# willSapgreen/stereo-vision

Measured on AMD Instinct MI355X. Metric: stereo pairs/sec (ELAS 1242x375, ROBOTICS, D1+D2+LR), higher is better.
Workload: dtype u8

## Files before the change

### include/svh.h

```cpp
#ifndef SVH_H
#define SVH_H

#include <stddef.h>
#include <stdint.h>

#ifdef __cplusplus
extern "C" {
#endif

#define SVH_OK                 0
#define SVH_ERR_FEW_SUPPORT    1
#define SVH_ERR_BAD_ARG       -1
#define SVH_ERR_HIP           -2
#define SVH_ERR_UNSUPPORTED   -3
#define SVH_ERR_NO_DEVICE     -4
#define SVH_ERR_BAD_DIMS      -7

typedef struct svh_elas_params {
    int32_t disp_min;
    int32_t disp_max;
    float   support_threshold;
    int32_t support_texture;
    int32_t candidate_stepsize;
    int32_t incon_window_size;
// ... 103 lines not shown
                                      uint64_t* first_ticket);
int32_t svh_elas_stream_pop_n(svh_elas_stream* s, int32_t n, int32_t* status, int32_t* popped);
int32_t svh_elas_stream_push_n(svh_elas_stream* s, int32_t n, const uint8_t* const* I1, const uint8_t* const* I2,
                               float* const* D1, float* const* D2, uint64_t* first_ticket);

#define SVH_DISP_F32 0
#define SVH_DISP_U16 1
#define SVH_MAPS_BOTH 0
#define SVH_MAPS_LEFT 1
typedef struct { int32_t format; int32_t maps; } svh_elas_output;
int32_t svh_elas_process_out(svh_elas* e, const uint8_t* I1, const uint8_t* I2, void* D1, void* D2,
                             const int32_t* dims, const svh_elas_output* out);
int32_t svh_elas_process_batch_out(svh_elas* e, int32_t n, const uint8_t* const* I1, const uint8_t* const* I2,
                                   void* const* D1, void* const* D2, const int32_t* dims, int32_t* status,
                                   const svh_elas_output* out);
svh_elas_stream* svh_elas_stream_open_out(svh_elas* e, const int32_t* dims, int32_t depth, const svh_elas_output* out);
int32_t svh_elas_stream_push_out(svh_elas_stream* s, const uint8_t* I1, const uint8_t* I2, void* D1, void* D2,
                                 uint64_t* ticket);
int32_t svh_elas_stream_push_out_n(svh_elas_stream* s, int32_t n, const uint8_t* const* I1, const uint8_t* const* I2,
                                   void* const* D1, void* const* D2, uint64_t* first_ticket);
int32_t svh_disparity_pack_u16(const float* D, int32_t d_on_device, int64_t n, uint16_t* out, int32_t out_on_device);
int32_t svh_disparity_unpack_u16(const uint16_t* v, int64_t n, float* out);

int64_t svh_elas_trim(void);

int32_t svh_elas_set_lanes(int32_t lanes);
int32_t svh_elas_set_queue_plan(int32_t plan);
int32_t svh_elas_get_queue_plan(int32_t* plan, int32_t* streams_per_lane, int32_t* classes);
int32_t svh_elas_set_group(int32_t pairs);

int32_t svh_elas_set_stage(int32_t where);
void svh_elas_stage_stats(int64_t* device_groups, int64_t* handed_back);
void svh_elas_sizing_stats(int64_t* out4);
void svh_elas_get_settings(int32_t out[4]);

enum svh_elas_stage {
    SVH_ELAS_DESC1 = 0,
    SVH_ELAS_DESC2,
    SVH_ELAS_DCAN_RAW,
    SVH_ELAS_SUPPORT,
    SVH_ELAS_TRI1,
    SVH_ELAS_TRI2,
    SVH_ELAS_PLANES1,
    SVH_ELAS_PLANES2,
    SVH_ELAS_GRID1,
    SVH_ELAS_GRID2,
    SVH_ELAS_D1_RAW,
    SVH_ELAS_D2_RAW,
    SVH_ELAS_D1_LR,
    SVH_ELAS_D2_LR,
    SVH_ELAS_D1_SEG,
    SVH_ELAS_D2_SEG,
    SVH_ELAS_D1_GAP,
    SVH_ELAS_D2_GAP,
    SVH_ELAS_STAGE_COUNT
};
int32_t svh_elas_set_taps(svh_elas* e, int32_t enable);
int32_t svh_elas_get_stage(svh_elas* e, int32_t stage, void* buf, size_t cap, size_t* size);

int32_t svh_elas_last_timing(svh_elas* e, const char** names, float* ms, int32_t cap);

int32_t svh_profile_enable(int32_t on);
void    svh_profile_only(const char* kernel);
void    svh_profile_reset(void);
int32_t svh_profile_get(int32_t index, const char** name, double* total_ms, int64_t* launches);

// ... 178 lines not shown
```

### stereo-vision_amd/csrc/elas_engine.cpp

```cpp
#include <hip/hip_runtime.h>
#include <stdio.h>
#include <string.h>

#include <atomic>
#include <chrono>
#include <condition_variable>
#include <deque>
#include <functional>
#include <algorithm>
#include <map>
#include <memory>
#include <mutex>
#include <string>
#include <thread>
#include <vector>

#include "hip_guard.h"
#include "queue_plan.h"
#include "svh_internal.h"

namespace svh {

static thread_local int t_device = 0;

#define HIP_TRY(kind, expr) SVH_HIP_TRY(nullptr, kind, expr)
#define LANE_GROW(buf, bytes) SVH_HIP_GROW(nullptr, buf, bytes)

struct KernelStat {
    double total_ms = 0;
    int64_t launches = 0;
};
static std::mutex g_prof_mu;
static std::map<std::string, KernelStat> g_prof;
static std::atomic<int> g_prof_on{0};
static char g_prof_only[64] = "";

struct EventProfiler : Profiler {
    hipStream_t stream = nullptr;
    std::vector<hipEvent_t> ev;
    std::vector<const char*> names;
    size_t used = 0;
    bool skipping = false;
    void begin(const char* kernel) override {
        skipping = g_prof_only[0] && strcmp(kernel, g_prof_only) != 0;
        if (skipping) return;
        if (ev.size() < 2 * (used + 1)) {
            hipEvent_t a, b;
            if (hipEventCreate(&a) != hipSuccess || hipEventCreate(&b) != hipSuccess) return;
            ev.push_back(a);
// ... 36 lines not shown

static int queue_cap();
static int worker_count();

struct LaneBufs {
    HipBuf<uint8_t> img;
    HipBuf<uint8_t> desc;
    HipBuf<int16_t> dcan;
    HipBuf<int32_t> owner;
    HipBuf<uint8_t> prior_dev;
    HipBuf<TriRaster> raster;
    HipBuf<float> planes;
    HipBuf<uint32_t> seed, mask;
    HipBuf<uint16_t> lists;
    HipBuf<float> Draw;
    HipBuf<float> D;
    HipBuf<float> tmp;
    HipBuf<uint16_t> U;
    HipBuf<int32_t> labels, counts;
    HipBuf<int32_t> seg_nroots;
    HipBuf<uint8_t> stage_blob;
    PinnedBuf<int16_t> h_dcan;
    PinnedBuf<uint8_t> h_img, h_prior;
    PinnedBuf<StageCounts> h_counts;
};

struct Lane : LaneBufs {
    EventProfiler prof;
    int device = 0;
    hipStream_t stream = nullptr, stage_stream = nullptr, post_stream = nullptr;
    hipStream_t cls_stream[QC_COUNT] = {nullptr, nullptr, nullptr};
    int plan_req = QP_AUTO;
    int parity = 0;
    bool qp_known = false;
    QueuePlan qp{};
    int prio_least = 0, prio_greatest = 0;
    bool split = false;
    hipEvent_t a_ev = nullptr, b_ev = nullptr;
    hipEvent_t wait_ev = nullptr;
    hipStream_t copy_stream = nullptr;
    hipEvent_t match_ev = nullptr, copy_ev = nullptr;
    bool poll_wait = false;
    bool parallel_host = true;
    bool lone_group = true;
    int32_t W = 0, H = 0, disp_max = -1, step = 0, grid_size = 0, sub = -1, gcap = 0;
    Dims d{};
    bool desc_fly = false;
    int64_t owner_hi = 0;
    size_t prior_cap = 0;
    size_t ntri_max = 0;
    std::vector<HostPrior> hp;
    std::vector<int32_t> P;
    StageDev stg{};
    bool stage_ok = false;
    hipEvent_t stage_ev = nullptr;
    bool resident = false;
    bool force_host = false;
    float P_key[5] = {-1, -1, -1, -1, -1};
    static constexpr int kHist = 4;
    int32_t hist_sup[kHist] = {}, hist_tri[kHist] = {};
    int hist_n = 0, hist_at = 0;
    int32_t hist_g = 0;
    svh_elas_params hist_p{};
    PhaseBSize sized{};
    size_t o_P = 0, o_sup = 0, o_tri = 0;

    void release() {
        if (!stream) return;
        (void)hipSetDevice(device);
        static_cast<LaneBufs&>(*this) = LaneBufs();
        stage_ok = false; stg = StageDev{};
        P_key[0] = -1;
        hist_n = 0;
        W = H = 0;
    }

    void destroy() {
        if (!cls_stream[QC_NORMAL] && !cls_stream[QC_HIGH] && !cls_stream[QC_LOW]) return;
        (void)hipSetDevice(device);
        release();
        for (hipEvent_t* e : {&wait_ev, &match_ev, &copy_ev, &stage_ev, &a_ev, &b_ev})
            if (*e) {
                (void)hipEventDestroy(*e);
                *e = nullptr;
            }
        for (hipEvent_t e : prof.ev) (void)hipEventDestroy(e);
        prof.ev.clear();
        prof.names.clear();
        if (copy_stream) (void)hipStreamDestroy(copy_stream);
        for (hipStream_t& cs : cls_stream)
            if (cs) {
                (void)hipStreamDestroy(cs);
                cs = nullptr;
            }
        copy_stream = stream = stage_stream = post_stream = nullptr;
    }

    int bind_streams() {
        if (!qp_known) {
            HIP_TRY(none, hipSetDevice(device));
            if (hipDeviceGetStreamPriorityRange(&prio_least, &prio_greatest) != hipSuccess) {
                (void)hipGetLastError();
                prio_least = prio_greatest = 0;
            }
            qp = make_queue_plan(prio_least, prio_greatest, queue_cap(), worker_count(), plan_req);
            qp_known = true;
        }
        const QueueLane& ql = qp.lane[parity & 1];
        for (int k = 0; k < ql.nstreams; k++) {
            hipStream_t& cs = cls_stream[ql.cls[k]];
            if (cs) continue;
            HIP_TRY(none, hipSetDevice(device));
            if (qp.plan == QP_ONE)
                HIP_TRY(none, hipStreamCreateWithFlags(&cs, hipStreamNonBlocking));
            else
                HIP_TRY(none, hipStreamCreateWithPriority(&cs, hipStreamNonBlocking,
                                                          queue_priority_of(ql.cls[k], prio_least, prio_greatest)));
        }
        stream = cls_stream[ql.cls[ql.phase_stream[QPH_A]]];
        stage_stream = cls_stream[ql.cls[ql.phase_stream[QPH_S]]];
        post_stream = cls_stream[ql.cls[ql.phase_stream[QPH_B]]];
        return SVH_OK;
    }

    int ensure(const svh_elas_params& p, int32_t w, int32_t h, int32_t g) {
        if (int rc = bind_streams()) return rc;
        const int32_t st = p.candidate_stepsize + (p.subsampling ? p.candidate_stepsize % 2 : 0);
        if (w == W && h == H && p.disp_max == disp_max && st == step && p.grid_size == grid_size &&
            p.subsampling == sub && g <= gcap)
            return SVH_OK;
        release();
        d = make_dims(p, w, h);
        const size_t N = (size_t)w * h, DN = (size_t)d.DW * d.DH, G2 = (size_t)2 * g;
        LANE_GROW(img, G2 * N);
        LANE_GROW(desc, G2 * N * 16);
        LANE_GROW(owner, G2 * N * sizeof(int32_t));
        HIP_TRY(copy, hipMemset(owner, 0, G2 * N * sizeof(int32_t)));
        owner_hi = svh::env("SVH_TEST_OWNER_HI") ? atoll(svh::env("SVH_TEST_OWNER_HI")) : 0;
        LANE_GROW(Draw, G2 * DN * sizeof(float));
        LANE_GROW(D, G2 * DN * sizeof(float));
        LANE_GROW(tmp, G2 * DN * sizeof(float));
        LANE_GROW(labels, G2 * DN * sizeof(int32_t));
        LANE_GROW(counts, G2 * DN * sizeof(int32_t));
        LANE_GROW(seg_nroots, G2 * (size_t)((d.DW + 63) / 64) * ((d.DH + 15) / 16) * sizeof(int32_t));
        const size_t nc = (size_t)d.Wc * d.Hc;
        LANE_GROW(dcan, g * nc * sizeof(int16_t));
        LANE_GROW(h_dcan, g * nc * sizeof(int16_t));
        LANE_GROW(h_img, G2 * N);
        const size_t nsup = nc + 6;
        ntri_max = 2 * nsup + 8;
// ... 24 lines not shown
            LANE_GROW(stage_blob, off);
            HIP_TRY(copy, hipMemset(stage_blob, 0, off));
            LANE_GROW(h_counts, sizeof(StageCounts));
            uint8_t* b = stage_blob;
            stg.dcan = dcan;
            stg.sup_raw = reinterpret_cast<int32_t*>(b + a_sup);
            stg.counts = reinterpret_cast<StageCounts*>(b + a_cnt);
            stg.ids = reinterpret_cast<int32_t*>(b + a_ids);
            stg.xys = reinterpret_cast<int32_t*>(b + a_xys);
            stg.nbr = reinterpret_cast<uint32_t*>(b + a_nbr);
            int32_t** ia[6] = {&stg.pxy, &stg.buck, &stg.buck2, &stg.byx, &stg.order, &stg.oxy};
            uint32_t** ua[4] = {&stg.lx, &stg.ly, &stg.tmp, &stg.P};
            for (int k = 0; k < 6; k++) *ia[k] = reinterpret_cast<int32_t*>(b + a_arr[k]);
            for (int k = 0; k < 4; k++) *ua[k] = reinterpret_cast<uint32_t*>(b + a_arr[6 + k]);
            stg.dmap = reinterpret_cast<int32_t*>(b + a_arr[10]);
            stg.fl = reinterpret_cast<uint32_t*>(b + a_fl);
            stg.fr = reinterpret_cast<uint32_t*>(b + a_fr);
            stg.wl = reinterpret_cast<int32_t*>(b + a_wl);
            stg.cntw = reinterpret_cast<uint32_t*>(b + a_cw);
            stg.sup_cap = (int32_t)cap;
            stg.rec_cap = (int32_t)rec;
            stage_ok = true;
        }
        HIP_TRY(wait, hipDeviceSynchronize());
        W = w; H = h; disp_max = p.disp_max; step = st; grid_size = p.grid_size; sub = p.subsampling;
        gcap = g;
        return SVH_OK;
    }
};

static std::atomic<int> g_wait_us{40};
static std::atomic<bool> g_hostprof{false};
static hipError_t lane_wait(Lane& L) {
    if (!L.poll_wait || g_wait_us <= 0) return hipStreamSynchronize(L.stream);
    if (!L.wait_ev) {
        hipError_t e = hipEventCreateWithFlags(&L.wait_ev, hipEventDisableTiming);
        if (e != hipSuccess) return e;
    }
    hipError_t e = hipEventRecord(L.wait_ev, L.stream);
    if (e != hipSuccess) return e;
    for (;;) {
        e = hipEventQuery(L.wait_ev);
        if (e != hipErrorNotReady) return e;
        std::this_thread::sleep_for(std::chrono::microseconds(g_wait_us.load(std::memory_order_relaxed)));
    }
}

struct Pool {
    std::mutex mu;
    std::condition_variable cv;
    std::vector<Lane*> lanes;
    std::vector<Lane*> free_list;
    int max_lanes = 4;
    int queue_plan = -2;
};

static std::mutex g_mu;

static std::map<int, Pool*>& g_pools = *new std::map<int, Pool*>();
static std::atomic<int> g_lanes{6};
static std::atomic<int> g_group{32};
static std::atomic<bool> g_group_set{false};
static std::atomic<int> g_stage_mode{-1};
static int stage_mode_from_env();
static std::atomic<int> g_queue_plan{QP_AUTO};
static std::atomic<int> g_queue_cap{kQueueCapDefault};
static int queue_cap() { return g_queue_cap.load(); }
static int worker_count() { return g_lanes.load(); }
static void apply_config(const svh_config& c, int explicit_call) {
    if (explicit_call) {
        if (c.elas_workers > 0) svh_elas_set_lanes(c.elas_workers);
        if (c.elas_pairs_per_launch > 0) svh_elas_set_group(c.elas_pairs_per_launch);
        svh_elas_set_stage(c.elas_stage);
        if (c.wait_us >= 0) g_wait_us = c.wait_us;
    }
    if (const char* e = svh::env("SVH_WAIT_US")) g_wait_us = atoi(e);
    if (svh::env("SVH_STAGE")) g_stage_mode.store(stage_mode_from_env());
    g_hostprof = svh::env("SVH_HOST_PROF") != nullptr;
    g_queue_cap = queue_cap_from_text(getenv("GPU_MAX_HW_QUEUES"));
    if (const char* e = svh::env("SVH_QUEUE_PLAN")) {
        const int v = atoi(e);
        g_queue_plan = v >= 0 && v <= QP_LAST ? v : QP_AUTO;
    }
}
namespace { struct ConfigHook { ConfigHook() { svh::on_config(apply_config); } } g_config_hook; }
static int group_for(size_t N) {
    const int g = std::max(1, std::min(g_group.load(), kMaxGroup));
    if (g_group_set.load()) return g;
    size_t a = std::max<size_t>(1, std::min<size_t>(g, (size_t)32 * 1024 * 1024 / std::max<size_t>(N, 1)));
    size_t free_b = 0, total_b = 0;
    if (a > 1 && hipMemGetInfo(&free_b, &total_b) == hipSuccess && free_b > 0) {
        const size_t per_pair = 120 * std::max<size_t>(N, 1), sets = (size_t)2 * std::max(1, g_lanes.load());
        a = std::max<size_t>(1, std::min<size_t>(a, free_b / 2 / (per_pair * sets)));
    } else {
        (void)hipGetLastError();
    }
    return (int)a;
}

static Pool* pool_for(int device) {
    std::lock_guard<std::mutex> lk(g_mu);
    auto it = g_pools.find(device);
    if (it != g_pools.end()) return it->second;
    Pool* p = new Pool();
    g_pools[device] = p;
    return p;
}

static void acquire_lanes(int device, int count, Lane** out) {
    Pool* p = pool_for(device);
    std::unique_lock<std::mutex> lk(p->mu);
    p->max_lanes = 2 * g_lanes.load() + 2;
    for (;;) {
        const int can_make = p->max_lanes - (int)p->lanes.size();
        if ((int)p->free_list.size() + std::max(can_make, 0) >= count) {
            for (int i = 0; i < count; i++) {
                if (!p->free_list.empty()) {
                    out[i] = p->free_list.back();
                    p->free_list.pop_back();
                } else {
                    Lane* l = new Lane();
                    l->device = device;
                    l->plan_req = p->queue_plan != -2 ? p->queue_plan : g_queue_plan.load();
                    p->lanes.push_back(l);
                    out[i] = l;
                }
                out[i]->parity = i;
            }
            return;
        }
        p->cv.wait(lk);
    }
}

static Lane* acquire_lane(int device) {
    Lane* l = nullptr;
    acquire_lanes(device, 1, &l);
    return l;
}

static void release_lane(Lane* l) {
    Pool* p = pool_for(l->device);
    {
        std::lock_guard<std::mutex> lk(p->mu);
        p->free_list.push_back(l);
    }
    p->cv.notify_all();
}

struct Taps {
    bool enabled = false;
    std::vector<uint8_t> data[SVH_ELAS_STAGE_COUNT];
};

}

struct svh_elas {
    svh_elas_params p;
    int device;
    svh::Taps taps;
    std::vector<std::string> tnames;
    std::vector<float> tms;
};

namespace svh {

struct GroupIO {
    int32_t g;
    bool in_device;
    const uint8_t* dI[2];
    size_t in_stride;
    const uint8_t* const* hI[2];
    int32_t pitch;
    bool out_device;
    float* dD[2];
    size_t out_stride;
    float* const* hD[2];
    int32_t format = SVH_DISP_F32;
// ... 39 lines not shown
static std::atomic<uint64_t> g_hp_ns[HP_N];
static std::atomic<uint64_t> g_hp_pairs{0};
static uint64_t cpu_ns() {
    timespec ts;
    clock_gettime(CLOCK_THREAD_CPUTIME_ID, &ts);
    return (uint64_t)ts.tv_sec * 1000000000ull + ts.tv_nsec;
}
struct HostProfDump {
    ~HostProfDump() {
        if (!g_hostprof || !g_hp_pairs) return;
        static const char* nm[HP_N] = {"enqueue A", "waits", "filters", "delaunay", "pack", "enqueue B"};
        double tot = 0;
        for (int i = 0; i < HP_N; i++) tot += g_hp_ns[i];
        fprintf(stderr, "[svh host prof] %llu pairs, %.1f us cpu/pair:", (unsigned long long)g_hp_pairs.load(),
                tot / 1e3 / g_hp_pairs);
        for (int i = 0; i < HP_N; i++) fprintf(stderr, "  %s %.1f", nm[i], g_hp_ns[i] / 1e3 / g_hp_pairs);
        fprintf(stderr, "\n");
    }
};
static HostProfDump g_hp_dump;
#define HP_MARK(slot) do { if (g_hostprof) { uint64_t n_ = cpu_ns(); g_hp_ns[slot] += n_ - hp_t; hp_t = n_; } } while (0)

static int stage_mode_from_env() {
    const char* e = svh::env("SVH_STAGE");
    if (!e || !*e || !strcmp(e, "auto") || !strcmp(e, "-1")) return -1;
    if (!strcmp(e, "host") || !strcmp(e, "0")) return 0;
    if (!strcmp(e, "device") || !strcmp(e, "1")) return 1;
    fprintf(stderr, "svhip: SVH_STAGE=%s is not one of auto|-1, host|0, device|1: using auto\n", e);
    return -1;
}

static std::atomic<int64_t> g_stage_dev_groups{0}, g_stage_redo_groups{0};
static std::atomic<int64_t> g_sized_bound{0}, g_sized_hist{0}, g_short_tri{0}, g_short_sup{0};

static hipError_t event_wait(Lane& L, hipEvent_t ev) {
    if (!L.poll_wait || g_wait_us <= 0) return hipEventSynchronize(ev);
    for (;;) {
        hipError_t e = hipEventQuery(ev);
        if (e != hipErrorNotReady) return e;
        std::this_thread::sleep_for(std::chrono::microseconds(g_wait_us.load(std::memory_order_relaxed)));
    }
}

static int run_group_body(Lane& L, const svh_elas_params& p, const int32_t* dims, const GroupIO& io,
                          int32_t* status, Taps* taps, svh_elas* timing, int mode, int prefer_device);

static int run_group(Lane& L, const svh_elas_params& p, const int32_t* dims, const GroupIO& io,
                     int32_t* status, Taps* taps, svh_elas* timing, int mode = RG_ALL, int prefer_device = 0) {
    const int rc = run_group_body(L, p, dims, io, status, taps, timing, mode, prefer_device);
    if (rc == SVH_ERR_HIP) {
        const std::string keep = svh_last_error();
        for (hipStream_t cs : L.cls_stream)
            if (cs) (void)hipStreamSynchronize(cs);
        L.split = false;
        if (L.copy_stream) (void)hipStreamSynchronize(L.copy_stream);
        (void)hipGetLastError();
        L.prof.used = 0;
        L.resident = false;
        L.force_host = false;
        L.P_key[0] = -1;
        fail(rc, keep);
    }
    return rc;
}

static int run_group_body(Lane& L, const svh_elas_params& p, const int32_t* dims, const GroupIO& io,
                          int32_t* status, Taps* taps, svh_elas* timing, int mode, int prefer_device) {
    const int32_t W = dims[0], H = dims[1], g = io.g;
    int rc = check_params(p, W, H);
    if (rc) return rc;
    if (g < 1 || g > kMaxGroup) return fail(SVH_ERR_BAD_ARG, "bad group size");
    HIP_TRY(none, hipSetDevice(L.device));
    rc = L.ensure(p, W, H, g);
    if (rc) return rc;
    if (g > 1) taps = nullptr;
    const Dims& d = L.d;
    const bool u16 = !io.out_device && io.format == SVH_DISP_U16;
    const int nmaps = !io.out_device && io.maps == SVH_MAPS_LEFT ? 1 : 2;
    const size_t DNu = ((size_t)d.DW * d.DH + 7) & ~(size_t)7;
    if (u16) LANE_GROW(L.U, (size_t)L.gcap * 2 * DNu * sizeof(uint16_t));
    hipStream_t s = L.stream, ss = s, sb = L.split ? L.post_stream : s;
    const bool prof_on = g_prof_on.load() != 0;
    PhaseProfiler prof_a(&L.prof, s), prof_s(&L.prof, s), prof_b(&L.prof, sb);
    const LaunchCtx cx = {s, prof_on ? &prof_a : nullptr, L.lone_group};
    LaunchCtx cx_s = cx, cx_b = {sb, prof_on ? &prof_b : nullptr, L.lone_group};
    const size_t N = (size_t)W * H, DN = (size_t)d.DW * d.DH;
    const size_t nc = (size_t)d.Wc * d.Hc;
// ... 582 lines not shown
}

void svh_profile_reset(void) {
    std::lock_guard<std::mutex> lk(g_prof_mu);
    g_prof.clear();
}

int32_t svh_profile_get(int32_t index, const char** name, double* total_ms, int64_t* launches) {
    std::lock_guard<std::mutex> lk(g_prof_mu);
    if (index < 0) return (int32_t)g_prof.size();
    int32_t i = 0;
    for (auto& kv : g_prof) {
        if (i++ == index) {
            if (name) *name = kv.first.c_str();
            if (total_ms) *total_ms = kv.second.total_ms;
            if (launches) *launches = kv.second.launches;
            return SVH_OK;
        }
    }
    return SVH_ERR_BAD_ARG;
}

int64_t svh_elas_trim(void) {
    int64_t freed = 0;
    std::vector<Pool*> pools;
    {
        std::lock_guard<std::mutex> lk(g_mu);
        for (auto& kv : g_pools) pools.push_back(kv.second);
    }
    for (Pool* p : pools) {
        std::vector<Lane*> idle;
        {
            std::lock_guard<std::mutex> lk(p->mu);
            idle.swap(p->free_list);
            for (Lane* l : idle) p->lanes.erase(std::find(p->lanes.begin(), p->lanes.end(), l));
        }
        for (Lane* l : idle) {
            l->destroy();
            delete l;
            freed++;
        }
        p->cv.notify_all();
    }
    return freed;
}

int32_t svh_elas_set_lanes(int32_t lanes) {
    if (lanes < 1) lanes = 1;
    if (lanes > 64) lanes = 64;
    g_lanes.store(lanes);
    return lanes;
}

void svh_elas_params_default(svh_elas_params* p, int32_t setting) {
    const bool rob = setting == SVH_ELAS_ROBOTICS;
    p->disp_min = 0;
    p->disp_max = 255;
    p->support_threshold = rob ? 0.85f : 0.95f;
    p->support_texture = 10;
    p->candidate_stepsize = 5;
    p->incon_window_size = 5;
    p->incon_threshold = 5;
    p->incon_min_support = 5;
    p->add_corners = rob ? 0 : 1;
    p->grid_size = 20;
    p->beta = 0.02f;
    p->gamma = rob ? 3.f : 5.f;
// ... 72 lines not shown
    rc = run_group(*L, e->p, dims, io, &st, &e->taps, e);
    release_lane(L);
    if (rc == SVH_ERR_HIP) report_hip_failure("svh_elas_process");
    return rc ? rc : st;
}

int32_t svh_elas_process(svh_elas* e, const uint8_t* I1, const uint8_t* I2, float* D1, float* D2,
                         const int32_t* dims) {
    if (!e || !I1 || !I2 || !D1 || !D2 || !dims) return fail(SVH_ERR_BAD_ARG, "null argument");
    return process_impl(e, I1, I2, D1, D2, dims, SVH_DISP_F32, SVH_MAPS_BOTH);
}

int32_t svh_elas_process_out(svh_elas* e, const uint8_t* I1, const uint8_t* I2, void* D1, void* D2,
                             const int32_t* dims, const svh_elas_output* out) {
    int32_t format, maps;
    if (!output_form(out, &format, &maps)) return fail(SVH_ERR_BAD_ARG, "bad output format / map selection");
    if (!e || !I1 || !I2 || !D1 || (!D2 && maps == SVH_MAPS_BOTH) || !dims) return fail(SVH_ERR_BAD_ARG, "null argument");
    return process_impl(e, I1, I2, static_cast<float*>(D1), static_cast<float*>(D2), dims, format, maps);
}

static int32_t batch_impl(svh_elas* e, int32_t n, const int32_t* dims, int32_t* status,
                          const std::function<GroupIO(int32_t, int32_t)>& io_of) {
    int32_t rc = require_device(e->device);
    if (rc) return rc;
    rc = check_params(e->p, dims[0], dims[1]);
    if (rc) return rc;
    const int32_t G = group_for((size_t)dims[0] * dims[1]);
    const int32_t ngroups = (n + G - 1) / G;
    const int lanes = std::min<int>(g_lanes.load(), ngroups);
    const int deep = n >= 32 ? 2 : 1;
    std::vector<int32_t> st(n, SVH_OK);
    std::vector<int32_t> grc(ngroups, SVH_OK);
    std::vector<std::string> errs(std::max(lanes, 1));
    auto worker = [&](int w) {
        Lane* slot[2] = {nullptr, nullptr};
        acquire_lanes(e->device, ngroups > 1 ? 2 : 1, slot);
        for (Lane* L : slot)
            if (L) {
                L->parallel_host = ngroups <= lanes;
                L->lone_group = ngroups == 1;
                L->poll_wait = !L->parallel_host;
                if (hipSetDevice(L->device) == hipSuccess) (void)L->ensure(e->p, dims[0], dims[1], G);
            }
        struct Job { int32_t gi = -1; GroupIO io{}; int32_t first = 0; };
        int32_t my_next = w;
        auto take = [&]() {
            Job j;
            const int32_t gi = my_next;
            my_next += lanes;
            if (gi < ngroups) {
                j.gi = gi;
                j.first = gi * G;
                j.io = io_of(j.first, std::min(G, n - j.first));
            }
            return j;
        };
        auto note = [&](const Job& j, int rcj) {
            if (rcj != SVH_OK && grc[j.gi] == SVH_OK) {
                grc[j.gi] = rcj;
                if (rcj < 0) errs[w] = svh_last_error();
            }
        };
        Job pending[2];
        Job cur = take();
        int k = 0;
        if (cur.gi >= 0) note(cur, run_group(*slot[0], e->p, dims, cur.io, &st[cur.first], nullptr, nullptr, RG_A, deep));
        while (cur.gi >= 0) {
            Job nxt = slot[1] ? take() : Job();
            if (nxt.gi >= 0) {
                const int o = 1 - k;
                if (pending[o].gi >= 0) {
                    note(pending[o], run_group(*slot[o], e->p, dims, pending[o].io, &st[pending[o].first], nullptr,
                                               nullptr, RG_FINISH));
                    pending[o].gi = -1;
                }
                note(nxt, run_group(*slot[o], e->p, dims, nxt.io, &st[nxt.first], nullptr, nullptr, RG_A, deep));
            }
            if (grc[cur.gi] == SVH_OK)
                note(cur, run_group(*slot[k], e->p, dims, cur.io, &st[cur.first], nullptr, nullptr, RG_HOST_B));
            pending[k] = cur;
            if (!slot[1]) {
                note(cur, run_group(*slot[0], e->p, dims, cur.io, &st[cur.first], nullptr, nullptr, RG_FINISH));
                pending[0].gi = -1;
                nxt = take();
                if (nxt.gi >= 0)
                    note(nxt, run_group(*slot[0], e->p, dims, nxt.io, &st[nxt.first], nullptr, nullptr, RG_A, deep));
            } else {
                k = 1 - k;
            }
            cur = nxt;
        }
        for (int q = 0; q < 2; q++)
            if (slot[q]) {
                if (pending[q].gi >= 0)
                    note(pending[q], run_group(*slot[q], e->p, dims, pending[q].io, &st[pending[q].first], nullptr,
                                               nullptr, RG_FINISH));
                slot[q]->poll_wait = false;
                slot[q]->parallel_host = true;
                slot[q]->lone_group = true;
                release_lane(slot[q]);
            }
    };
    if (lanes <= 1) {
        worker(0);
    } else {
        std::atomic<int> left{lanes - 1};
        const int dev = e->device;
        for (int w = 1; w < lanes; w++)
            crew().post([&, w, dev]() {
                t_device = dev;
                worker(w);
                left.fetch_sub(1, std::memory_order_release);
            });
        worker(0);
        crew().wait(left);
    }
    int32_t first_bad = SVH_OK;
    for (int32_t gi = 0; gi < ngroups; gi++)
        if (grc[gi] != SVH_OK) {
            for (int32_t i = gi * G; i < std::min(n, (gi + 1) * G); i++) st[i] = grc[gi];
        }
    for (int32_t i = 0; i < n; i++) {
        if (status) status[i] = st[i];
        if (first_bad == SVH_OK && st[i] != SVH_OK) first_bad = st[i];
    }
    for (auto& m : errs)
        if (!m.empty()) fail(first_bad, m);
    if (first_bad == SVH_ERR_HIP) report_hip_failure("svh_elas_process_batch");
    return first_bad;
}

static int32_t batch_host(svh_elas* e, int32_t n, const uint8_t* const* I1, const uint8_t* const* I2,
                          float* const* D1, float* const* D2, const int32_t* dims, int32_t* status, int32_t format,
                          int32_t maps) {
    if (n == 0) return SVH_OK;
    return batch_impl(e, n, dims, status, [&](int32_t first, int32_t cnt) {
        GroupIO io{};
        io.g = cnt;
        io.in_device = false;
        io.hI[0] = I1 + first; io.hI[1] = I2 + first; io.pitch = dims[2];
        io.out_device = false;
        io.hD[0] = D1 + first; io.hD[1] = D2 ? D2 + first : nullptr;
        io.format = format; io.maps = maps;
        return io;
    });
}

int32_t svh_elas_process_batch(svh_elas* e, int32_t n, const uint8_t* const* I1,
                               const uint8_t* const* I2, float* const* D1, float* const* D2,
// ... 372 lines not shown
    const int32_t n = (int32_t)(s.size() / 3);
    for (int32_t i = 0; i < n && i < cap; i++)
        for (int k = 0; k < 3; k++) support[3 * i + k] = s[3 * i + k];
    return n;
}


int32_t svh_elas_set_stage(int32_t where) {
    g_stage_mode.store(where < 0 ? -1 : (where ? 1 : 0));
    return g_stage_mode.load();
}

void svh_debug_stage_stamps(int64_t* out32) {
    Pool* p = pool_for(t_device);
    std::lock_guard<std::mutex> lk(p->mu);
    for (Lane* l : p->lanes)
        if (l->stage_ok) {
            (void)hipMemcpy(out32, l->stg.counts->dbg, 32 * sizeof(int64_t), hipMemcpyDeviceToHost);
            return;
        }
}

void svh_test_d2h_map_bytes(int64_t out[2], int32_t reset) {
    if (out) {
        out[0] = svh::g_d2h_map_bytes.load();
        out[1] = svh::g_d2h_map_copies.load();
    }
    if (reset) {
        svh::g_d2h_map_bytes.store(0);
        svh::g_d2h_map_copies.store(0);
    }
}

void svh_elas_sizing_stats(int64_t* out4) {
    if (!out4) return;
    out4[0] = svh::g_sized_bound.load();
    out4[1] = svh::g_sized_hist.load();
    out4[2] = svh::g_short_tri.load();
    out4[3] = svh::g_short_sup.load();
}

void svh_elas_stage_stats(int64_t* device_groups, int64_t* handed_back) {
    if (device_groups) *device_groups = g_stage_dev_groups.load();
    if (handed_back) *handed_back = g_stage_redo_groups.load();
}

void svh_elas_get_settings(int32_t out[4]) {
    if (!out) return;
    out[0] = g_lanes.load();
    out[1] = g_group_set.load() ? g_group.load() : 0;
    out[2] = g_stage_mode.load();
    out[3] = g_wait_us;
}

int32_t svh_elas_set_queue_plan(int32_t plan) {
    svh::ensure_init();
    if (plan < 0 || plan > QP_LAST) plan = QP_AUTO;
    Pool* p = pool_for(t_device);
    std::lock_guard<std::mutex> lk(p->mu);
    p->queue_plan = plan;
    return plan;
}

int32_t svh_elas_get_queue_plan(int32_t* plan, int32_t* streams_per_lane, int32_t* classes) {
    svh::ensure_init();
    Pool* p = pool_for(t_device);
// ... 28 lines not shown
```

### stereo-vision_amd/svhip/__init__.py

```python
import ctypes as C
import os

import numpy as np

_HERE = os.path.dirname(os.path.abspath(__file__))
LIB_PATH = os.environ.get("SVH_LIB") or os.path.join(os.path.dirname(_HERE), "libsvhip.so")

OK, ERR_FEW_SUPPORT, ERR_BAD_ARG, ERR_HIP, ERR_UNSUPPORTED, ERR_NO_DEVICE = 0, 1, -1, -2, -3, -4
ERR_BAD_DIMS = -7
ROBOTICS, MIDDLEBURY = 0, 1


class ElasParams(C.Structure):
    _fields_ = [
        ("disp_min", C.c_int32), ("disp_max", C.c_int32),
        ("support_threshold", C.c_float), ("support_texture", C.c_int32),
        ("candidate_stepsize", C.c_int32), ("incon_window_size", C.c_int32),
        ("incon_threshold", C.c_int32), ("incon_min_support", C.c_int32),
        ("add_corners", C.c_int32), ("grid_size", C.c_int32),
        ("beta", C.c_float), ("gamma", C.c_float), ("sigma", C.c_float), ("sradius", C.c_float),
        ("match_texture", C.c_int32), ("lr_threshold", C.c_int32),
        ("speckle_sim_threshold", C.c_float), ("speckle_size", C.c_int32),
        ("ipol_gap_width", C.c_int32), ("filter_median", C.c_int32),
        ("filter_adaptive_mean", C.c_int32), ("postprocess_only_left", C.c_int32),
# ... 365 lines not shown
            if rc < 0:
                raise SvhError(rc, last_error())
        return buf.view(dtype)

    def last_timing(self):
        names = (C.c_char_p * 16)()
        ms = (C.c_float * 16)()
        n = lib().svh_elas_last_timing(self._h, names, ms, 16)
        return [(names[i].decode(), ms[i]) for i in range(n)]


def set_lanes(n):
    return lib().svh_elas_set_lanes(n)


def set_group(n):
    return lib().svh_elas_set_group(n)


def set_stage(where):
    return lib().svh_elas_set_stage(where)


def set_queue_plan(plan):
    return lib().svh_elas_set_queue_plan(int(plan))


def queue_plan():
    p, s, c = C.c_int32(-9), C.c_int32(-9), C.c_int32(-9)
    lib().svh_elas_get_queue_plan(C.byref(p), C.byref(s), C.byref(c))
    return dict(plan=p.value, streams_per_lane=s.value, classes=c.value)


def trim():
    lib().svh_elas_trim.restype = C.c_int64
    return lib().svh_elas_trim()


def stage_stats():
    a, b = C.c_int64(0), C.c_int64(0)
    lib().svh_elas_stage_stats(C.byref(a), C.byref(b))
    return a.value, b.value


def device_count():
    return lib().svh_device_count()


def pack_u16(D):
    D = np.ascontiguousarray(D, np.float32)
    out = np.empty(D.shape, np.uint16)
    rc = lib().svh_disparity_pack_u16(D.ctypes.data, 0, D.size, out.ctypes.data, 0)
    if rc < 0:
        raise SvhError(rc, last_error())
    return out


def unpack_u16(v):
    v = np.ascontiguousarray(v, np.uint16)
    out = np.empty(v.shape, np.float32)
    rc = lib().svh_disparity_unpack_u16(v.ctypes.data, v.size, out.ctypes.data)
    if rc < 0:
        raise SvhError(rc, last_error())
    return out


# ... 454 lines not shown
```

Before: 36830.

## Dynamically feed groups to workers and drive lanes with a non-blocking state machine

Workers now take their first group by worker index and later groups from a shared atomic counter, replacing the fixed round-robin split, so faster workers can absorb leftover groups. Each worker's two lanes are driven by a polling state machine that records an event after the host-side B phase and finishes whichever lane completes first, instead of strictly alternating. Free lanes are kept in per-parity lists so the queue-priority parity of a lane is preserved when it is reused, and lanes of the wrong parity may be retired and rebuilt. The polling loop adds sleep-based spinning, lane churn and extra stats counters, which could add host overhead or contention.

Result: faster. 38840 (median of 6 runs) (+5.4%).

```diff
diff --git a/include/svh.h b/include/svh.h
--- a/include/svh.h
+++ b/include/svh.h
@@ -159,6 +159,9 @@
 int32_t svh_elas_set_stage(int32_t where);
 void svh_elas_stage_stats(int64_t* device_groups, int64_t* handed_back);
 void svh_elas_sizing_stats(int64_t* out4);
+#define SVH_ELAS_FEED_WORKERS 64
+#define SVH_ELAS_FEED_STATS_LEN (8 + 2 * SVH_ELAS_FEED_WORKERS)
+void svh_elas_feed_stats(int64_t* out);
 void svh_elas_get_settings(int32_t out[4]);
 
 enum svh_elas_stage {
diff --git a/stereo-vision_amd/csrc/elas_engine.cpp b/stereo-vision_amd/csrc/elas_engine.cpp
--- a/stereo-vision_amd/csrc/elas_engine.cpp
+++ b/stereo-vision_amd/csrc/elas_engine.cpp
@@ -15,6 +15,7 @@
 #include <thread>
 #include <vector>
 
+#include "group_feed.h"
 #include "hip_guard.h"
 #include "queue_plan.h"
 #include "svh_internal.h"
@@ -117,12 +118,15 @@
     hipStream_t cls_stream[QC_COUNT] = {nullptr, nullptr, nullptr};
     int plan_req = QP_AUTO;
     int parity = 0;
+    uint64_t freed_at = 0;
+    std::atomic<int>* cls_count = nullptr;
     bool qp_known = false;
     QueuePlan qp{};
     int prio_least = 0, prio_greatest = 0;
     bool split = false;
     hipEvent_t a_ev = nullptr, b_ev = nullptr;
     hipEvent_t wait_ev = nullptr;
+    bool wait_marked = false;
     hipStream_t copy_stream = nullptr;
     hipEvent_t match_ev = nullptr, copy_ev = nullptr;
     bool poll_wait = false;
@@ -173,10 +177,11 @@
         prof.ev.clear();
         prof.names.clear();
         if (copy_stream) (void)hipStreamDestroy(copy_stream);
-        for (hipStream_t& cs : cls_stream)
-            if (cs) {
-                (void)hipStreamDestroy(cs);
-                cs = nullptr;
+        for (int c = 0; c < QC_COUNT; c++)
+            if (cls_stream[c]) {
+                (void)hipStreamDestroy(cls_stream[c]);
+                cls_stream[c] = nullptr;
+                if (cls_count) cls_count[c].fetch_sub(1, std::memory_order_relaxed);
             }
         copy_stream = stream = stage_stream = post_stream = nullptr;
     }
@@ -201,6 +206,7 @@
             else
                 HIP_TRY(none, hipStreamCreateWithPriority(&cs, hipStreamNonBlocking,
                                                           queue_priority_of(ql.cls[k], prio_least, prio_greatest)));
+            if (cls_count) cls_count[ql.cls[k]].fetch_add(1, std::memory_order_relaxed);
         }
         stream = cls_stream[ql.cls[ql.phase_stream[QPH_A]]];
         stage_stream = cls_stream[ql.cls[ql.phase_stream[QPH_S]]];
@@ -291,13 +297,21 @@
 static std::atomic<int> g_wait_us{40};
 static std::atomic<bool> g_hostprof{false};
 static hipError_t lane_wait(Lane& L) {
-    if (!L.poll_wait || g_wait_us <= 0) return hipStreamSynchronize(L.stream);
+    if (!L.poll_wait || g_wait_us <= 0) {
+        L.wait_marked = false;
+        return hipStreamSynchronize(L.stream);
+    }
     if (!L.wait_ev) {
         hipError_t e = hipEventCreateWithFlags(&L.wait_ev, hipEventDisableTiming);
         if (e != hipSuccess) return e;
     }
-    hipError_t e = hipEventRecord(L.wait_ev, L.stream);
-    if (e != hipSuccess) return e;
+    hipError_t e = hipSuccess;
+    if (L.wait_marked) {
+        L.wait_marked = false;
+    } else {
+        e = hipEventRecord(L.wait_ev, L.stream);
+        if (e != hipSuccess) return e;
+    }
     for (;;) {
         e = hipEventQuery(L.wait_ev);
         if (e != hipErrorNotReady) return e;
@@ -305,11 +319,25 @@
     }
 }
 
+static void lane_mark(Lane& L) {
+    if (!L.poll_wait || g_wait_us <= 0) return;
+    if (!L.wait_ev && hipEventCreateWithFlags(&L.wait_ev, hipEventDisableTiming) != hipSuccess) {
+        (void)hipGetLastError();
+        L.wait_ev = nullptr;
+        return;
+    }
+    if (hipEventRecord(L.wait_ev, L.stream) == hipSuccess) L.wait_marked = true;
+    else (void)hipGetLastError();
+}
+static bool lane_done(Lane& L) { return !L.wait_marked || hipEventQuery(L.wait_ev) != hipErrorNotReady; }
+
 struct Pool {
     std::mutex mu;
     std::condition_variable cv;
     std::vector<Lane*> lanes;
-    std::vector<Lane*> free_list;
+    std::vector<Lane*> free_list[2];
+    uint64_t freed = 0;
+    std::atomic<int> streams[QC_COUNT] = {};
     int max_lanes = 4;
     int queue_plan = -2;
 };
@@ -366,30 +394,82 @@
     return p;
 }
 
-static void acquire_lanes(int device, int count, Lane** out) {
+static int feed_mode() { return feed_mode_from_text(svh::env("SVH_FEED")); }
+
+static Lane* make_lane(Pool* p, int device, int parity) {
+    Lane* l = new Lane();
+    l->device = device;
+    l->parity = parity;
+    l->plan_req = p->queue_plan != -2 ? p->queue_plan : g_queue_plan.load();
+    l->cls_count = p->streams;
+    p->lanes.push_back(l);
+    return l;
+}
+
+static void acquire_lanes(int device, int count, Lane** out, int feed = -1) {
+    if (feed < 0) feed = feed_mode();
     Pool* p = pool_for(device);
-    std::unique_lock<std::mutex> lk(p->mu);
-    p->max_lanes = 2 * g_lanes.load() + 2;
-    for (;;) {
-        const int can_make = p->max_lanes - (int)p->lanes.size();
-        if ((int)p->free_list.size() + std::max(can_make, 0) >= count) {
-            for (int i = 0; i < count; i++) {
-                if (!p->free_list.empty()) {
-                    out[i] = p->free_list.back();
-                    p->free_list.pop_back();
+    Lane* retired[2] = {nullptr, nullptr};
+    {
+        std::unique_lock<std::mutex> lk(p->mu);
+        p->max_lanes = 2 * g_lanes.load() + 2;
+        std::vector<Lane*>* fl = p->free_list;
+        for (;; p->cv.wait(lk)) {
+            const int can_make = std::max(p->max_lanes - (int)p->lanes.size(), 0);
+            if (feed & FEED_PARITY_AT_ACQUIRE) {
+                if ((int)(fl[0].size() + fl[1].size()) + can_make < count) continue;
+                for (int i = 0; i < count; i++) {
+                    int q = -1;
+                    for (int c = 0; c < 2; c++)
+                        if (!fl[c].empty() && (q < 0 || fl[c].back()->freed_at > fl[q].back()->freed_at)) q = c;
+                    if (q >= 0) {
+                        out[i] = fl[q].back();
+                        fl[q].pop_back();
+                    } else {
+                        out[i] = make_lane(p, device, i);
+                    }
+                    out[i]->parity = i;
+                }
+                break;
+            }
+            if (count == 1) {
+                const int q = !fl[0].empty() ? 0 : can_make > 0 ? -1 : !fl[1].empty() ? 1 : -2;
+                if (q == -2) continue;
+                if (q < 0) {
+                    out[0] = make_lane(p, device, 0);
                 } else {
-                    Lane* l = new Lane();
-                    l->device = device;
-                    l->plan_req = p->queue_plan != -2 ? p->queue_plan : g_queue_plan.load();
-                    p->lanes.push_back(l);
-                    out[i] = l;
+                    out[0] = fl[q].back();
+                    fl[q].pop_back();
                 }
-                out[i]->parity = i;
-            }
-            return;
-        }
-        p->cv.wait(lk);
-    }
+                break;
+            }
+            const int missing = (int)fl[0].empty() + (int)fl[1].empty();
+            int spare = 0;
+            for (int q = 0; q < 2; q++) spare += std::max((int)fl[q].size() - 1, 0);
+            if (missing > can_make + spare) continue;
+            for (int q = 0; q < 2; q++) {
+                if (!fl[q].empty()) {
+                    out[q] = fl[q].back();
+                    fl[q].pop_back();
+                    continue;
+                }
+                if (p->max_lanes <= (int)p->lanes.size()) {
+                    std::vector<Lane*>& from = fl[1 - q];
+                    Lane* victim = from.front();
+                    from.erase(from.begin());
+                    p->lanes.erase(std::find(p->lanes.begin(), p->lanes.end(), victim));
+                    retired[q] = victim;
+                }
+                out[q] = make_lane(p, device, q);
+            }
+            break;
+        }
+    }
+    for (Lane* l : retired)
+        if (l) {
+            l->destroy();
+            delete l;
+        }
 }
 
 static Lane* acquire_lane(int device) {
@@ -402,7 +482,8 @@
     Pool* p = pool_for(l->device);
     {
         std::lock_guard<std::mutex> lk(p->mu);
-        p->free_list.push_back(l);
+        l->freed_at = ++p->freed;
+        p->free_list[l->parity & 1].push_back(l);
     }
     p->cv.notify_all();
 }
@@ -508,6 +589,9 @@
 
 static std::atomic<int64_t> g_stage_dev_groups{0}, g_stage_redo_groups{0};
 static std::atomic<int64_t> g_sized_bound{0}, g_sized_hist{0}, g_short_tri{0}, g_short_sup{0};
+constexpr int kFeedWorkers = 64;
+static std::atomic<int64_t> g_feed_workers{0}, g_feed_groups{0}, g_feed_call_us{0}, g_feed_out_of_turn{0};
+static std::atomic<int64_t> g_feed_taken[kFeedWorkers], g_feed_finish_us[kFeedWorkers];
 
 static hipError_t event_wait(Lane& L, hipEvent_t ev) {
     if (!L.poll_wait || g_wait_us <= 0) return hipEventSynchronize(ev);
@@ -529,6 +613,7 @@
         for (hipStream_t cs : L.cls_stream)
             if (cs) (void)hipStreamSynchronize(cs);
         L.split = false;
+        L.wait_marked = false;
         if (L.copy_stream) (void)hipStreamSynchronize(L.copy_stream);
         (void)hipGetLastError();
         L.prof.used = 0;
@@ -1177,7 +1262,9 @@
         std::vector<Lane*> idle;
         {
             std::lock_guard<std::mutex> lk(p->mu);
-            idle.swap(p->free_list);
+            idle.swap(p->free_list[0]);
+            idle.insert(idle.end(), p->free_list[1].begin(), p->free_list[1].end());
+            p->free_list[1].clear();
             for (Lane* l : idle) p->lanes.erase(std::find(p->lanes.begin(), p->lanes.end(), l));
         }
         for (Lane* l : idle) {
@@ -1316,9 +1403,18 @@
     std::vector<int32_t> st(n, SVH_OK);
     std::vector<int32_t> grc(ngroups, SVH_OK);
     std::vector<std::string> errs(std::max(lanes, 1));
+    const int feed_bits = feed_mode();
+    GroupFeed feed;
+    const auto call_t0 = std::chrono::steady_clock::now();
+    auto call_us = [&]() {
+        return (int64_t)std::chrono::duration_cast<std::chrono::microseconds>(std::chrono::steady_clock::now() - call_t0).count();
+    };
+    g_feed_workers = std::max(lanes, 1);
+    g_feed_groups = ngroups;
+    for (int w = 0; w < kFeedWorkers; w++) g_feed_taken[w] = g_feed_finish_us[w] = 0;
     auto worker = [&](int w) {
         Lane* slot[2] = {nullptr, nullptr};
-        acquire_lanes(e->device, ngroups > 1 ? 2 : 1, slot);
+        acquire_lanes(e->device, ngroups > 1 ? 2 : 1, slot, feed_bits);
         for (Lane* L : slot)
             if (L) {
                 L->parallel_host = ngroups <= lanes;
@@ -1327,12 +1423,15 @@
                 if (hipSetDevice(L->device) == hipSuccess) (void)L->ensure(e->p, dims[0], dims[1], G);
             }
         struct Job { int32_t gi = -1; GroupIO io{}; int32_t first = 0; };
-        int32_t my_next = w;
+        const bool fixed = (feed_bits & FEED_FIXED_SHARES) != 0;
+        const int nworkers = std::max(lanes, 1);
+        FeedCursor cursor;
+        auto more = [&]() { return feed_peek(feed, cursor, fixed, w, nworkers, ngroups) >= 0; };
         auto take = [&]() {
             Job j;
-            const int32_t gi = my_next;
-            my_next += lanes;
-            if (gi < ngroups) {
+            const int32_t gi = feed_take(feed, cursor, fixed, w, nworkers, ngroups);
+            if (gi >= 0) {
+                if (w < kFeedWorkers) g_feed_taken[w].fetch_add(1, std::memory_order_relaxed);
                 j.gi = gi;
                 j.first = gi * G;
                 j.io = io_of(j.first, std::min(G, n - j.first));
@@ -1345,8 +1444,69 @@
                 if (rcj < 0) errs[w] = svh_last_error();
             }
         };
+        auto finished = [&]() {
+            if (w < kFeedWorkers) g_feed_finish_us[w].store(call_us(), std::memory_order_relaxed);
+        };
         Job pending[2];
-        Job cur = take();
+        if (!(feed_bits & FEED_ALTERNATE)) {
+            enum { LS_EMPTY = 0, LS_A = 1, LS_ALL = 2 };
+            int state[2] = {LS_EMPTY, LS_EMPTY};
+            const int nl = slot[1] ? 2 : 1;
+            int last_filled = -1;
+            auto start = [&](int q) {
+                Job j = take();
+                if (j.gi < 0) return false;
+                if (nl == 2 && q == last_filled) g_feed_out_of_turn.fetch_add(1, std::memory_order_relaxed);
+                last_filled = q;
+                note(j, run_group(*slot[q], e->p, dims, j.io, &st[j.first], nullptr, nullptr, RG_A, deep));
+                pending[q] = j;
+                state[q] = LS_A;
+                return true;
+            };
+            auto host_b = [&](int q) {
+                const Job& j = pending[q];
+                if (grc[j.gi] == SVH_OK) {
+                    note(j, run_group(*slot[q], e->p, dims, j.io, &st[j.first], nullptr, nullptr, RG_HOST_B));
+                    if (grc[j.gi] == SVH_OK) lane_mark(*slot[q]);
+                }
+                state[q] = LS_ALL;
+            };
+            auto finish = [&](int q) {
+                const Job& j = pending[q];
+                note(j, run_group(*slot[q], e->p, dims, j.io, &st[j.first], nullptr, nullptr, RG_FINISH));
+                finished();
+                pending[q].gi = -1;
+                state[q] = LS_EMPTY;
+            };
+            auto stage_ready = [&](Lane& L) {
+                return !L.poll_wait || g_wait_us <= 0 || hipEventQuery(L.stage_ev) != hipErrorNotReady;
+            };
+            for (;;) {
+                bool progress = false;
+                for (int q = 0; q < nl; q++) {
+                    if (state[q] == LS_ALL && lane_done(*slot[q])) {
+                        finish(q);
+                        progress = true;
+                    }
+                    if (state[q] == LS_EMPTY && start(q)) progress = true;
+                    if (state[q] != LS_A) continue;
+                    Lane& L = *slot[q];
+                    if (grc[pending[q].gi] != SVH_OK || !L.resident) {
+                        const int o = 1 - q;
+                        if (nl == 2 && state[o] == LS_ALL && more()) finish(o);
+                        if (nl == 2 && state[o] == LS_EMPTY) start(o);
+                        host_b(q);
+                        progress = true;
+                    } else if (pending[q].io.out_device || stage_ready(L)) {
+                        host_b(q);
+                        progress = true;
+                    }
+                }
+                if (state[0] == LS_EMPTY && state[nl - 1] == LS_EMPTY && !more()) break;
+                if (!progress) std::this_thread::sleep_for(std::chrono::microseconds(std::max(g_wait_us.load(std::memory_order_relaxed), 1)));
+            }
+        }
+        Job cur = (feed_bits & FEED_ALTERNATE) ? take() : Job();
         int k = 0;
         if (cur.gi >= 0) note(cur, run_group(*slot[0], e->p, dims, cur.io, &st[cur.first], nullptr, nullptr, RG_A, deep));
         while (cur.gi >= 0) {
@@ -1356,6 +1516,7 @@
                 if (pending[o].gi >= 0) {
                     note(pending[o], run_group(*slot[o], e->p, dims, pending[o].io, &st[pending[o].first], nullptr,
                                                nullptr, RG_FINISH));
+                    finished();
                     pending[o].gi = -1;
                 }
                 note(nxt, run_group(*slot[o], e->p, dims, nxt.io, &st[nxt.first], nullptr, nullptr, RG_A, deep));
@@ -1365,6 +1526,7 @@
             pending[k] = cur;
             if (!slot[1]) {
                 note(cur, run_group(*slot[0], e->p, dims, cur.io, &st[cur.first], nullptr, nullptr, RG_FINISH));
+                finished();
                 pending[0].gi = -1;
                 nxt = take();
                 if (nxt.gi >= 0)
@@ -1376,9 +1538,11 @@
         }
         for (int q = 0; q < 2; q++)
             if (slot[q]) {
-                if (pending[q].gi >= 0)
+                if (pending[q].gi >= 0) {
                     note(pending[q], run_group(*slot[q], e->p, dims, pending[q].io, &st[pending[q].first], nullptr,
                                                nullptr, RG_FINISH));
+                    finished();
+                }
                 slot[q]->poll_wait = false;
                 slot[q]->parallel_host = true;
                 slot[q]->lone_group = true;
@@ -1399,6 +1563,7 @@
         worker(0);
         crew().wait(left);
     }
+    g_feed_call_us = call_us();
     int32_t first_bad = SVH_OK;
     for (int32_t gi = 0; gi < ngroups; gi++)
         if (grc[gi] != SVH_OK) {
@@ -1837,6 +2002,27 @@
     }
 }
 
+void svh_elas_feed_stats(int64_t* out) {
+    if (!out) return;
+    for (int i = 0; i < SVH_ELAS_FEED_STATS_LEN; i++) out[i] = 0;
+    out[0] = svh::g_feed_workers.load();
+    out[1] = svh::g_feed_groups.load();
+    out[2] = svh::g_feed_call_us.load();
+    out[3] = svh::g_feed_out_of_turn.load();
+    {
+        Pool* p = pool_for(t_device);
+        std::lock_guard<std::mutex> lk(p->mu);
+        out[4] = (int64_t)p->lanes.size();
+        out[5] = p->streams[QC_NORMAL].load();
+        out[6] = p->streams[QC_HIGH].load();
+        out[7] = p->streams[QC_LOW].load();
+    }
+    for (int w = 0; w < svh::kFeedWorkers && w < SVH_ELAS_FEED_WORKERS; w++) {
+        out[8 + 2 * w] = svh::g_feed_taken[w].load();
+        out[9 + 2 * w] = svh::g_feed_finish_us[w].load();
+    }
+}
+
 void svh_elas_sizing_stats(int64_t* out4) {
     if (!out4) return;
     out4[0] = svh::g_sized_bound.load();
diff --git a/stereo-vision_amd/csrc/group_feed.h b/stereo-vision_amd/csrc/group_feed.h
--- /dev/null
+++ b/stereo-vision_amd/csrc/group_feed.h
@@ -0,0 +1,49 @@
+#ifndef SVH_GROUP_FEED_H
+#define SVH_GROUP_FEED_H
+
+#include <stdint.h>
+
+#include <atomic>
+
+namespace svh {
+
+enum {
+    FEED_PARITY_AT_ACQUIRE = 1,
+    FEED_FIXED_SHARES = 2,
+    FEED_ALTERNATE = 4,
+    FEED_ALL = 7,
+};
+inline int feed_mode_from_text(const char* text) {
+    if (!text || !*text) return 0;
+    int v = 0;
+    for (const char* c = text; *c >= '0' && *c <= '9' && v < 1000; c++) v = v * 10 + (*c - '0');
+    return v & FEED_ALL;
+}
+
+struct GroupFeed {
+    std::atomic<int32_t> next{0};
+};
+struct FeedCursor {
+    int32_t taken = 0;
+};
+
+inline int32_t feed_peek(const GroupFeed& f, const FeedCursor& c, bool fixed, int w, int workers, int32_t ngroups) {
+    if (workers < 1 || w < 0 || w >= workers) return -1;
+    int64_t gi;
+    if (fixed || c.taken == 0) gi = (int64_t)w + (int64_t)c.taken * workers;
+    else gi = (int64_t)workers + f.next.load(std::memory_order_relaxed);
+    return gi < ngroups ? (int32_t)gi : -1;
+}
+
+inline int32_t feed_take(GroupFeed& f, FeedCursor& c, bool fixed, int w, int workers, int32_t ngroups) {
+    if (feed_peek(f, c, fixed, w, workers, ngroups) < 0) return -1;
+    int64_t gi;
+    if (fixed || c.taken == 0) gi = (int64_t)w + (int64_t)c.taken * workers;
+    else gi = (int64_t)workers + f.next.fetch_add(1, std::memory_order_relaxed);
+    if (gi >= ngroups) return -1;
+    c.taken++;
+    return (int32_t)gi;
+}
+
+}
+#endif
diff --git a/stereo-vision_amd/svhip/__init__.py b/stereo-vision_amd/svhip/__init__.py
--- a/stereo-vision_amd/svhip/__init__.py
+++ b/stereo-vision_amd/svhip/__init__.py
@@ -421,6 +421,17 @@
     return dict(plan=p.value, streams_per_lane=s.value, classes=c.value)
 
 
+def feed_stats():
+    nw = 64
+    out = (C.c_int64 * (8 + 2 * nw))()
+    lib().svh_elas_feed_stats(out)
+    w = int(out[0])
+    return dict(workers=w, groups=int(out[1]), call_us=int(out[2]), out_of_turn=int(out[3]), lanes=int(out[4]),
+                streams=dict(normal=int(out[5]), high=int(out[6]), low=int(out[7])),
+                taken=[int(out[8 + 2 * k]) for k in range(min(w, nw))],
+                finish_us=[int(out[9 + 2 * k]) for k in range(min(w, nw))])
+
+
 def trim():
     lib().svh_elas_trim.restype = C.c_int64
     return lib().svh_elas_trim()
```
